# clvrai/mopa-rl

Measured on AMD Instinct MI355X. Metric: valid-state collision checks/sec, higher is better.
Workload: dtype f64; 1 GPU; SawyerPushObstacle-v0 state validity (FK + collision), 4096 envs/GPU x 256 states/env per step, states 50% uniform joint-box samples + 50% near-init N(0,0.3); envs_per_gpu=4096, states_per_env=256, parallelism=env-shard x1

## Files before the change

### mopa_rl_amd/csrc/mopa_hip.hip

```cpp
#include <hip/hip_runtime.h>

#include <algorithm>
#include <cmath>
#include <cstdio>
#include <cstdlib>
#include <cstddef>
#include <cstring>
#include <string>
#include <utility>
#include <vector>

#include <map>
#include <mutex>
#include "../../include/mopa_hip.h"
#include "mopa_device.hpp"
#include "mopa_frames.hpp"
#include "mopa_manifold.hpp"
#include "mopa_sep.hpp"
#include "mopa_fk.hpp"
#include "mopa_host.hpp"
#include "mopa_model_host.hpp"

using namespace mopa;

// ... 154 lines not shown
}
MOPA_D bool wave_any(bool p) { return __ballot(p) != 0ull; }
MOPA_D double wave_min(double v) {
#pragma unroll
    for (int off = 32; off > 0; off >>= 1) {
        double o = __shfl_xor(v, off, 64);
        v = (o < v) ? o : v;
    }
    return v;
}

MOPA_D void tile_ctr_release(unsigned long long *ctr, int lane) {
    if (lane == 0) {
        const unsigned long long done = atomicAdd(ctr + 1, 1ull);
        if (done + 1ull == (unsigned long long)gridDim.x * (blockDim.x >> 6)) {
            atomicExch(ctr, 0ull);
            atomicExch(ctr + 1, 0ull);
        }
    }
}
MOPA_D long long wave_pull64(unsigned long long *ctr, int lane) {
    unsigned long long t = 0ull;
    if (lane == 0) t = atomicAdd(ctr, 1ull);
    const unsigned t_lo = __builtin_amdgcn_readfirstlane((unsigned)t), t_hi = __builtin_amdgcn_readfirstlane((unsigned)(t >> 32));
    return (long long)(((unsigned long long)t_hi << 32) | t_lo);
}
MOPA_D void wave_argmin(double &bd, int &bi) {
#pragma unroll
    for (int off = 32; off > 0; off >>= 1) {
        const double od = __shfl_xor(bd, off, 64);
        const int oi = __shfl_xor(bi, off, 64);
        if (od < bd || (od == bd && oi < bi)) { bd = od; bi = oi; }
    }
}
MOPA_D void row_fill_unused(int32_t *__restrict__ pair, double *__restrict__ dist, long long s, int K, int from, int lane) {
    for (int i = from + lane; i < K; i += 64) {
        pair[s * K + i] = -1;
        dist[s * K + i] = kFar;
    }
}

struct LdsView {
    const double *dbl;
    const int *ints;
    double *grec;
    double *qbuf;
    double *sc;
    unsigned short *wl;
};

MOPA_D void stage_scene(const SceneHdr &h, const double *g_dbl, const int32_t *g_int, double *s_dbl, int *s_int) {
    for (int i = threadIdx.x; i < h.n_dbl; i += blockDim.x) s_dbl[i] = g_dbl[i];
    for (int i = threadIdx.x; i < h.n_int; i += blockDim.x) s_int[i] = g_int[i];
    __syncthreads();
}

MOPA_D LdsView make_view(const SceneHdr &h, unsigned char *smem) {
    LdsView v;
    double *s_dbl = reinterpret_cast<double *>(smem);
    int *s_int = reinterpret_cast<int *>(s_dbl + h.n_dbl);
    int int_pad = (h.n_int + 1) & ~1;
    unsigned char *wave_base = reinterpret_cast<unsigned char *>(s_int + int_pad) + __builtin_amdgcn_readfirstlane((int)(threadIdx.x >> 6)) * h.wave_bytes;
    v.dbl = s_dbl;
    v.ints = s_int;
    v.grec = reinterpret_cast<double *>(wave_base);
    v.qbuf = v.grec + h.nmg * kGeomStride;
    v.sc = v.qbuf + h.na + h.n_pq + h.na;
    v.wl = reinterpret_cast<unsigned short *>(v.sc + 2 * h.nmj);
    return v;
}
MOPA_D LdsView global_view(const double *g_dbl, const int32_t *g_int) {
    LdsView v;
    v.dbl = g_dbl; v.ints = g_int; v.grec = nullptr; v.qbuf = nullptr; v.sc = nullptr; v.wl = nullptr;
    return v;
}

MOPA_D const double *geom_rec(const SceneHdr &h, const LdsView &v, int g) {
    int slot = v.ints[h.o_g_slot + g];
    return (slot >= 0) ? (v.grec + slot * kGeomStride) : (v.dbl + h.o_g_rec + g * kGeomStride);
}

MOPA_D bool pair_culled(const SceneHdr &h, const LdsView &v, int g1, int g2, const double *A, const double *B) {
    const int *I = v.ints;
    const double *D = v.dbl;
    const int t1 = I[h.o_g_type + g1];
    if (bp_cull(A, t1, D[h.o_g_rbound + g1], B, D[h.o_g_rbound + g2])) return true;
    if (t1 == G_PLANE) return false;
    const bool s1 = I[h.o_g_slot + g1] < 0, s2 = I[h.o_g_slot + g2] < 0;
    if (s1 == s2) return false;
    const int gs = s1 ? g1 : g2, gm = s1 ? g2 : g1;
    return aabb_cull(ld3((s1 ? A : B) + GO_POS), D + h.o_g_aabb + 3 * gs, ld3((s1 ? B : A) + GO_POS), D[h.o_g_rbound + gm]);
}
MOPA_D bool pair_culled_band(const SceneHdr &h, const LdsView &v, int g1, int g2, const double *A, const double *B, double band) {
    const int *I = v.ints;
    const double *D = v.dbl;
    const double rba = D[h.o_g_rbound + g1], rbb = D[h.o_g_rbound + g2];
    const V3 diff = sub3(ld3(B + GO_POS), ld3(A + GO_POS));
    if (I[h.o_g_type + g1] == G_PLANE) return dot3(diff, col3(A + GO_MAT, 2)) > rbb + band;
    const double rs = rba + rbb + band;
    if (dot3(diff, diff) > rs * rs) return true;
    const bool s1 = I[h.o_g_slot + g1] < 0, s2 = I[h.o_g_slot + g2] < 0;
    if (s1 == s2) return false;
    return aabb_cull(ld3((s1 ? A : B) + GO_POS), D + h.o_g_aabb + 3 * (s1 ? g1 : g2), ld3((s1 ? B : A) + GO_POS), (s1 ? rbb : rba) + band);
}
struct CullZeroMargin {
    MOPA_D bool operator()(const SceneHdr &h, const LdsView &v, int g1, int g2, const double *A, const double *B) const { return pair_culled(h, v, g1, g2, A, B); }
// ... 660 lines not shown
```

### mopa_rl_amd/csrc/mopa_valid_launch.inc

```

static int64_t k1_lane_min(const MopaScene *S) { return S->k1.v2_forced ? 64 : std::max<int64_t>(64, (int64_t)S->n_cu * 36); }
static int64_t k1_motion_expand_min(const MopaScene *S) { return S->k1.v2_forced ? 64 : std::max<int64_t>(64, (int64_t)S->n_cu * 16); }

using K1FnV1 = decltype(&k_is_valid<false, false>);
using K1FnV2 = decltype(&k_is_valid_v2<false, false>);
using K1FnV5 = decltype(&k_is_valid_v5<false, true, false>);
#define MOPA_K1_COUNT(i_, T_) +1
constexpr int kK1BakedScenes = 0 MOPA_K1_BAKED_SCENES(MOPA_K1_COUNT);
#undef MOPA_K1_COUNT

static K1FnV1 k1_kernel_v1(bool want_md, bool mesh) {
    static const K1FnV1 tab[2][2] = {{k_is_valid<false, false>, k_is_valid<true, false>}, {k_is_valid<false, true>, k_is_valid<true, true>}};
    return tab[mesh][want_md];
}
static K1FnV2 k1_kernel_v2(bool want_md, bool mesh) {
    static const K1FnV2 tab[2][2] = {{k_is_valid_v2<false, false>, k_is_valid_v2<true, false>}, {k_is_valid_v2<false, true>, k_is_valid_v2<true, true>}};
    return tab[mesh][want_md];
}
static K1FnV5 k1_kernel_v5(bool want_md, bool cen_lds, bool gate, int baked) {
    static const K1FnV5 generic[3][2] = {{k_is_valid_v5<false, true, false>, k_is_valid_v5<true, true, false>},
                                         {k_is_valid_v5<false, false, false>, k_is_valid_v5<true, false, false>},
                                         {k_is_valid_v5<false, false, true>, k_is_valid_v5<true, false, true>}};
    if (cen_lds && gate) return nullptr;
    if (!baked) return generic[cen_lds ? 0 : (gate ? 2 : 1)][want_md];
// ... 101 lines not shown
        p.wave = true;
        p.wave_grid = grid_for(S, v2_min);
        p.n_small = v2_min;
    }
    const int64_t tiles = (N + 63) / 64;
    p.blocks = std::min<int64_t>((tiles + kWavesPerBlock - 1) / kWavesPerBlock, (int64_t)S->n_cu * 2);
    p.waves = (size_t)p.blocks * kWavesPerBlock;
    p.v5 = P.use_v5 != 0;
    p.cen_lds = P.v5_cen_lds;
    p.baked = S->k1_baked;
    p.ent_cap = want_md ? P.v5_ent_cap_md : S->hdr.v5_ent_cap;
    if (p.baked) {
        const int ax = k1_baked_axis_words(p.baked) + k1_baked_pair_words(p.baked, want_md);
        if (p.ent_cap - ax >= 256) p.ent_cap -= ax;
        else if (ax > 0) p.baked = 0;
        p.tiles_per_drain = k1_baked_tiles_per_drain(p.baked, want_md);
        if (p.tiles_per_drain > 1) p.pair_tiles = std::max<long long>(0, (long long)tiles - (knobs.pair_tail_set ? std::max<long long>(0, knobs.pair_tail) : (long long)p.waves)) & ~1ll;
    }
    p.lane_lds = !p.v5 ? P.v2_lds_bytes : (want_md ? P.v5_lds_bytes_md : P.v5_lds_bytes);
    p.rows_cap = knobs.rows_cap_set ? knobs.rows_cap : std::min<long long>(std::max<long long>(4096, (long long)N / 2), 1ll << 22);
    p.gate = p.v5 && !p.cen_lds && S->n_mesh_gp > 0;
    p.rows = p.gate && p.rows_cap > 0;
    if (has_n_dev && S->n_mesh_gp > 0 && !p.gate) { p.refusal = "a device-side state count on a scene with mesh pairs needs the gated mesh pass"; return p; }
    p.rows_grid = (unsigned)(knobs.rows_blocks > 0 ? knobs.rows_blocks : 3 * S->n_cu);
    p.rows_lds = (int)((size_t)S->n_mesh_dbl * sizeof(double));
    p.mesh_pass = S->n_mesh_gp > 0;
    p.mesh_lds = P.v2_lds_bytes;
    const unsigned fb = knobs.fb_blocks > 0 ? (unsigned)knobs.fb_blocks : (p.rows ? (unsigned)std::max(1, S->n_cu / 4) : (unsigned)S->n_cu);
    p.mesh_grid = p.gate ? std::min<unsigned>((unsigned)p.blocks, fb) : (unsigned)p.blocks;
    p.debug_mesh = p.gate && knobs.debug_mesh;
    return p;
}

extern "C" int mopa_scene_valid_kernel(const MopaScene *S, int64_t N, char *out, int32_t cap) {
    if (!S || !out || cap < 24) return fail(MOPA_ERR_INVALID_ARG, "null argument / buffer under 24 bytes");
    const K1Plan p = k1_plan(S, N, false, false, false);
    std::snprintf(out, (size_t)cap, "%s", !p.lane ? "k_is_valid" : (p.v5 ? "k_is_valid_v5" : "k_is_valid_v2"));
    return MOPA_OK;
}
extern "C" int mopa_scene_k1_drain_plan(const MopaScene *S, int64_t N, int32_t want_md, int32_t *tiles_per_drain, int32_t *ent_cap) {
    if (!S || !tiles_per_drain || !ent_cap) return fail(MOPA_ERR_INVALID_ARG, "null argument");
    const K1Plan p = k1_plan(S, N, want_md != 0, false, false);
    const bool v5 = p.lane && p.v5;
    *tiles_per_drain = v5 ? p.tiles_per_drain : 0;
    *ent_cap = v5 ? p.ent_cap : 0;
    return MOPA_OK;
}
extern "C" int mopa_scene_motion_kernel(const MopaScene *S, int64_t N, char *out, int32_t cap) {
    if (!S || !out || cap < 24) return fail(MOPA_ERR_INVALID_ARG, "null argument / buffer under 24 bytes");
    std::snprintf(out, (size_t)cap, "%s", S->k1.use_v2 && N >= k1_motion_expand_min(S) ? "k_motion_expand" : "k_check_motion");
    return MOPA_OK;
}

static int launch_is_valid(MopaScene *S, const double *q_active, const double *qpos_env, int64_t N, int64_t samples_per_env,
                           const int *env_idx, uint8_t *valid, double *min_dist, void *stream, const long long *n_dev = nullptr,
                           bool attach = false) {
    if (!S || !valid || (N > 0 && (!q_active || !qpos_env))) return fail(MOPA_ERR_INVALID_ARG, "null argument");
    if (const int rc = state_batch_rule(N, samples_per_env)) return rc;
    if (N == 0) return MOPA_OK;
    ON_DEVICE(S->device);
    hipStream_t st = (hipStream_t)stream;
    if (attach && S->glue_b >= 0) {
        const int rc = glue_attach_scratch(S, qpos_env, (N + samples_per_env - 1) / samples_per_env, st, &qpos_env);
        if (rc) return rc;
    }
    dim3 block(kBlock);
    const K1Plan p = k1_plan(S, N, min_dist != nullptr, env_idx != nullptr, n_dev != nullptr);
    if (p.refusal) return fail(MOPA_ERR_UNSUPPORTED, p.refusal);
    if (p.wave) {
        hipLaunchKernelGGL(k1_kernel_v1(min_dist != nullptr, S->hdr.has_mesh != 0), dim3(p.wave_grid), block, p.wave_lds, st, S->hdr, S->d_dbl, S->d_int, q_active, qpos_env,
                           (long long)N, (long long)samples_per_env, valid, min_dist, env_idx, n_dev, p.lane ? p.n_small : (long long)(1ll << 62));
    }
    if (!p.lane) {
        HIP_TRY(hipGetLastError());
        return MOPA_OK;
    }
    StreamScratch &sc = scratch_for(S, st);
    if (p.waves > sc.slab_waves || (size_t)p.tiles_per_drain > sc.slab_tiles) {
        const size_t want = std::max(std::max(p.waves, sc.slab_waves), (size_t)S->n_cu * 2 * kWavesPerBlock);
        const size_t tiles = std::max((size_t)p.tiles_per_drain, sc.slab_tiles);
        HIP_TRY(grow(S, sc.slab, (want * tiles * (size_t)(S->hdr.nmg + S->hdr.n_save) * kSlabStride + 16) * sizeof(double)));
        HIP_TRY(grow(S, sc.mpr, want * (size_t)kMprCapV5 * kMprRow * sizeof(double)));
        HIP_TRY(grow(S, sc.cen, want * (size_t)S->hdr.nmg * 3 * 64 * sizeof(float)));
        sc.slab_waves = want;
        sc.slab_tiles = tiles;
    }
    if (!sc.k1_ctr.p) {
        HIP_TRY(grow(S, sc.k1_ctr, 64));
        HIP_TRY(hipMemset(sc.k1_ctr.p, 0, 64));
        HIP_TRY(hipStreamSynchronize(nullptr));
    }
    unsigned long long *const d_ctr = sc.k1_ctr.as<unsigned long long>();
    double *const d_slab = sc.slab.as<double>();
    dim3 grid((unsigned)p.blocks);
#ifdef MOPA_V2_PROFILE
    double *d_tail = d_slab + (size_t)p.blocks * kWavesPerBlock * p.tiles_per_drain * (S->hdr.nmg + S->hdr.n_save) * kSlabStride;
    unsigned long long *d_prof = (unsigned long long *)d_tail;
    (void)zero_async(d_prof, 6 * 8, st);
#endif
    long long *mesh_list = nullptr;
    unsigned long long *rows_cnt = nullptr;
    double *mesh_rows = nullptr;
    if (p.gate) {
        HIP_TRY(grow(S, sc.mesh_list, ((size_t)N + 2) * sizeof(long long)));
        rows_cnt = sc.mesh_list.as<unsigned long long>();
        mesh_list = sc.mesh_list.as<long long>() + 1;
        HIP_TRY(zero_async(rows_cnt, 2 * sizeof(long long), st));
        if (p.rows) {
            HIP_TRY(grow(S, sc.mesh_rows, (size_t)p.rows_cap * kMprRow * sizeof(double)));
            mesh_rows = sc.mesh_rows.as<double>();
        }
    }
    if (p.v5) {
        SceneHdr hk = S->hdr;
        hk.v5_ent_cap = p.ent_cap;
        hipLaunchKernelGGL(k1_kernel_v5(min_dist != nullptr, p.cen_lds, p.gate, p.baked), grid, block, p.lane_lds, st, hk, S->d_dbl, S->d_int, S->d_gp_tab, q_active, qpos_env,
                           (long long)N, (long long)samples_per_env, valid, min_dist, d_slab, env_idx, sc.mpr.as<double>(), mesh_list, sc.cen.as<float>(),
                           n_dev, d_ctr, mesh_rows, p.rows_cap, rows_cnt, p.n_small, p.pair_tiles);
        if (p.rows)
            hipLaunchKernelGGL(min_dist ? k_mesh_rows<true> : k_mesh_rows<false>, dim3(p.rows_grid), block, p.rows_lds, st, S->hdr, S->d_dbl, (const double *)mesh_rows,
                               (const unsigned long long *)rows_cnt, p.rows_cap, S->n_mesh_dbl, valid, min_dist);
    } else
        hipLaunchKernelGGL(k1_kernel_v2(min_dist != nullptr, false), grid, block, p.lane_lds, st, S->hdr, S->d_dbl, S->d_int, q_active, qpos_env, (long long)N,
                           (long long)samples_per_env, valid, min_dist, d_slab, 0, env_idx, (const long long *)nullptr, d_ctr);
    if (p.mesh_pass)
        hipLaunchKernelGGL(k1_kernel_v2(min_dist != nullptr, true), dim3(p.mesh_grid), block, p.mesh_lds, st, S->hdr_mesh, S->d_dbl, S->d_int, q_active, qpos_env, (long long)N,
                           (long long)samples_per_env, valid, min_dist, d_slab, 1, env_idx, (const long long *)mesh_list, d_ctr);
    HIP_TRY(hipGetLastError());
    if (p.debug_mesh) {
        long long cnt[2] = {0, 0};
        (void)hipStreamSynchronize(st);
        (void)hipMemcpy(cnt, mesh_list - 1, sizeof(cnt), hipMemcpyDeviceToHost);
        fprintf(stderr, "[mopa] mesh gate: %lld rows handed to k_mesh_rows (cap %lld), %lld of %lld states go to the second pass\n", cnt[0], p.rows_cap, cnt[1], (long long)N);
    }
#ifdef MOPA_V2_PROFILE
    {
        unsigned long long hp[6];
        (void)hipStreamSynchronize(st);
        (void)hipMemcpy(hp, d_prof, 48, hipMemcpyDeviceToHost);
        if (hp[5]) fprintf(stderr, "[v2 profile] per tile cycles: body %.0f geom %.0f cull+push %.0f flush %.0f total %.0f (tiles %llu)\n",
                           (double)hp[0] / hp[5], (double)hp[1] / hp[5], (double)hp[2] / hp[5], (double)hp[3] / hp[5], (double)hp[4] / hp[5], hp[5]);
    }
#endif
    return MOPA_OK;
}

extern "C" int mopa_is_valid_batch(MopaScene *S, const double *q_active, const double *qpos_env, int64_t N,
                                   int64_t samples_per_env, uint8_t *valid, double *min_dist, void *stream) {
    return launch_is_valid(S, q_active, qpos_env, N, samples_per_env, nullptr, valid, min_dist, stream, nullptr, true);
}
extern "C" int mopa_is_valid_batch_counted(MopaScene *S, const double *q_active, const double *qpos_env, int64_t N, int64_t samples_per_env,
// ... 5 lines not shown
```

### mopa_rl_amd/csrc/mopa_valid_v5.inc

```

constexpr int kEntCapV5Max = 1024;
constexpr int kBatCapV5 = 128;
constexpr int kMprCapV5 = 128;
constexpr int kMprRow = 32;
constexpr float kCullEps = 2.0e-5f;

MOPA_D unsigned long long v5_depth_image(double d) { return d != d ? 0x0007ffffffffffffull : f64_sortable(d); }

struct K1Generic {
    static constexpr bool kBaked = false;
    static constexpr int n_ax = 0;
    static constexpr int kTilesPerDrain = 1;
};
#include "mopa_valid_v5_baked.inc"

#ifdef MOPA_V5_TILES_PER_DRAIN
template <class TR, bool WANT_MD> constexpr int k1_tiles_per_drain = TR::kBaked && !WANT_MD ? MOPA_V5_TILES_PER_DRAIN : 1;
#else
template <class TR, bool WANT_MD> constexpr int k1_tiles_per_drain = WANT_MD ? 1 : TR::kTilesPerDrain;
#endif
constexpr unsigned kEntHalfBit = 31;
template <class TR, bool WANT_MD>
constexpr int k1_pair_words_of() {
    constexpr int T = k1_tiles_per_drain<TR, WANT_MD>;
// ... 257 lines not shown
        if constexpr (load == -2) {
            constexpr const unsigned long long *f = TR::fk_sf[sf];
            ppos = V3{k1_bits(f[0]), k1_bits(f[1]), k1_bits(f[2])};
            pquat = Q4{k1_bits(f[3]), k1_bits(f[4]), k1_bits(f[5]), k1_bits(f[6])};
#pragma unroll
            for (int i = 0; i < 9; i++) r.mat[i] = k1_bits(f[7 + i]);
        } else if constexpr (load >= 0) {
            ppos = r.save_pos[load];
            pquat = r.save_quat[load];
            quat2mat(r.mat, pquat);
        } else {
            ppos = r.pos;
            pquat = r.quat;
        }
        const V3 bp{k1_bits(bd[0]), k1_bits(bd[1]), k1_bits(bd[2])};
        const Q4 bq{k1_bits(bd[3]), k1_bits(bd[4]), k1_bits(bd[5]), k1_bits(bd[6])};
        if constexpr (SP) {
            r.pos = k1_offset_s<k1_kind(bd[0]), k1_kind(bd[1]), k1_kind(bd[2])>(ppos, r.mat, bp);
            r.quat = k1_quat_mul_s<k1_kind(bd[3]), k1_kind(bd[4]), k1_kind(bd[5]), k1_kind(bd[6])>(pquat, bq);
        } else {
            r.pos = add3(ppos, mat_vec(r.mat, bp));
            r.quat = quat_mul(pquat, bq);
        }
        if constexpr (jn == 1) {
            const V3 ax{k1_bits(bd[7]), k1_bits(bd[8]), k1_bits(bd[9])}, jp{k1_bits(bd[10]), k1_bits(bd[11]), k1_bits(bd[12])};
            constexpr double ref = k1_bits(bd[13]);
            constexpr int kax = k1_kind(bd[7]), kay = k1_kind(bd[8]), kaz = k1_kind(bd[9]);
            if constexpr (SP && jt == J_HINGE && jp0 && kax == KT_ZERO && kay == KT_ZERO && kaz == KT_ONE) {
                double s1, c1;
                if constexpr (src < TR::na) { s1 = sn[src]; c1 = cs[src]; }
                else mopa_sincos(0.5 * (pv[src - TR::na] - ref), s1, c1);
                r.quat = k1_quat_mul_s<KT_GEN, KT_ZERO, KT_ZERO, KT_GEN>(r.quat, Q4{c1, 0.0, 0.0, s1});
            } else if constexpr (SP && jt == J_SLIDE) {
                double dq;
                if constexpr (src < TR::na) dq = qact[src] - ref;
                else dq = pv[src - TR::na] - ref;
                double jm[9];
                quat2mat(jm, r.quat);
                r.pos = addscl3(r.pos, k1_mat_vec_s<kax, kay, kaz>(jm, ax), dq);
            } else {
                if constexpr (src < TR::na) apply_joint_sc(jt, ax, jp, jp0, qact[src] - ref, sn[src], cs[src], r.pos, r.quat);
                else apply_joint(jt, ax, jp, jp0, pv[src - TR::na] - ref, r.pos, r.quat);
            }
        }
        r.quat = quat_normalize(r.quat);
    }
    quat2mat(r.mat, r.quat);
    if constexpr (save >= 0) {
        r.save_pos[save] = r.pos;
        r.save_quat[save] = r.quat;
    }
    (k1_fk_geom<TR, mgadr + G, SP>(r, sink), ...);
}
template <class TR, bool SPARSE = false, class Sink, int... B>
MOPA_HD bool k1_fk_baked(const double *qa_row, const double *env_row, Sink &sink, std::integer_sequence<int, B...>) {
    static_assert(TR::na <= 8 && TR::n_pq >= 1 && TR::n_save >= 1, "baked walk: at most 8 active values; array sizes padded to 1");
    static_assert(TR::n_res <= kResMax, "baked walk: at most kResMax resident pairs");
    double qact[TR::na], pv[TR::n_pq], sn[TR::na], cs[TR::na];
#pragma unroll
    for (int a = 0; a < TR::na; a++) qact[a] = qa_row[a];
#pragma unroll
    for (int k = 0; k < TR::n_pq; k++) pv[k] = env_row[TR::fk_pq_adr[k]];
#pragma unroll
    for (int a = 0; a < TR::na; a++) mopa_sincos(0.5 * (qact[a] - k1_bits(TR::fk_act_ref[a])), sn[a], cs[a]);
    K1FkRegs<TR> r;
    r.pos = V3{0.0, 0.0, 0.0};
    r.quat = Q4{1.0, 0.0, 0.0, 0.0};
    r.trip = 0u;
    if constexpr (SPARSE) {
#pragma unroll
        for (int a = 0; a < TR::na; a++) r.trip |= !(fabs(qact[a]) <= kSparseInMax) ? 1u : 0u;
#pragma unroll
        for (int k = 0; k < TR::n_pq; k++) r.trip |= !(fabs(pv[k]) <= kSparseInMax) ? 1u : 0u;
        k1_pin(r.trip);
    }
    (k1_fk_body<TR, B, SPARSE>(r, qact, sn, cs, pv, sink, std::make_integer_sequence<int, TR::fk_body[B][4]>{}), ...);
    return r.trip != 0u;
}
template <bool COLD>
struct V5FkSinkT {
    double *slab;
    float *cen;
    MOPA_D void operator()(int m, V3 gp, Q4 gq) {
        double *sp = slab + (size_t)m * kSlabStride;
        if constexpr (COLD) asm volatile("" : "+v"(sp));
        pose7_st<64>(sp, gp, gq);
        float *cp = cen + (size_t)m * 3 * 64;
        cp[0] = (float)gp.x; cp[64] = (float)gp.y; cp[128] = (float)gp.z;
    }
    double res_d[kResMax];
    MOPA_D void resident(int r, double d) { res_d[r] = d; }
    int ax_row;
    MOPA_D void axis(int slot, unsigned word) { reinterpret_cast<unsigned *>(cen)[(ax_row + slot) * 64] = word; }
};
using V5FkSink = V5FkSinkT<false>;

struct V5Lds {
    float *cen;
    unsigned *ent;
    unsigned *bat;
    unsigned *bat2;
    unsigned long long *bad;
    unsigned long long *md;
    bool tp;
};
MOPA_HD int v5_lds_per_wave(int nmg, int ent_cap, bool want_md) { return ((nmg * 3 * 64 * 4) + ent_cap * 4 + 2 * kBatCapV5 * 4 + (want_md ? 64 * 8 : 0) + 8 + 15) & ~15; }

MOPA_D void v5_load_rec2(double (&R1)[15], double (&R2)[15], const SceneHdr &h, const double *D, const double *slab_tile,
                         int gA, int movA, int slotA, int gB, int movB, int slotB, int slA, int slB) {
    const double *sA = D + h.o_g_rec + gA * kGeomStride, *sB = D + h.o_g_rec + gB * kGeomStride;
    double a[7] = {0.0, 0.0, 0.0, 1.0, 0.0, 0.0, 0.0}, b[7] = {0.0, 0.0, 0.0, 1.0, 0.0, 0.0, 0.0};
    if (movA) {
        const double *sp = slab_tile + (size_t)slotA * kSlabStride + slA;
#pragma unroll
        for (int k = 0; k < 7; k++) a[k] = sp[64 * k];
    }
    if (movB) {
        const double *sp = slab_tile + (size_t)slotB * kSlabStride + slB;
#pragma unroll
        for (int k = 0; k < 7; k++) b[k] = sp[64 * k];
    }
#pragma unroll
    for (int i = 0; i < 15; i++) { R1[i] = sA[i]; R2[i] = sB[i]; }
    if (movA) {
        R1[0] = a[0]; R1[1] = a[1]; R1[2] = a[2];
        quat2mat(R1 + GO_MAT, Q4{a[3], a[4], a[5], a[6]});
    }
    if (movB) {
        R2[0] = b[0]; R2[1] = b[1]; R2[2] = b[2];
        quat2mat(R2 + GO_MAT, Q4{b[3], b[4], b[5], b[6]});
    }
}

template <bool WANT_MD, int T = 1>
MOPA_D int v5_flush(const SceneHdr &h, const LdsView &v, const V5Lds &q, const int *s_tab, const double *slab_tile, int lane,
                    int head, int n, int code, int stage = 0, int head2 = 0, int count2 = 0, double *mpr_ring = nullptr,
                    int mpr_head = 0, int *mpr_count = nullptr, long long tile_base = 0) {
    bool to_mpr = false;
    unsigned e = 0;
// ... 72 lines not shown

template <bool WANT_MD, int T = 1>
MOPA_D void v5_drain(const SceneHdr &h, const LdsView &v, const V5Lds &q, const int *s_tab, const double *slab_tile, int lane,
                     int n_ent, unsigned present, double *mpr_ring, int mpr_head, int *mpr_count, long long tile_base) {
    wave_sync();
    for (int code = 0; code < PC_COUNT; code++) {
        if (!((present >> code) & 1u)) continue;
        int head = 0, count = 0, head2 = 0, count2 = 0;
        for (int base = 0; base < n_ent; base += 64) {
            const int i = base + lane;
            bool take = false;
            unsigned e = 0;
            if (i < n_ent) {
                e = q.ent[i];
                take = (int)((e >> 12) & 0xf) == code;
                if (!WANT_MD) take = take && !((q.bad[T > 1 ? e >> kEntHalfBit : 0u] >> (e & 63)) & 1ull);
            }
            const unsigned long long mask = __ballot(take);
            if (!mask) continue;
            if (take) q.bat[(head + count + __popcll(mask & ((1ull << lane) - 1ull))) & (kBatCapV5 - 1)] = e;
            count += __popcll(mask);
            if (count >= 64) {
                wave_sync();
                if (code == PC_CONVEX) {
                    count2 += v5_flush<WANT_MD, T>(h, v, q, s_tab, slab_tile, lane, head, 64, code, 1, head2, count2, mpr_ring, mpr_head, mpr_count, tile_base);
                    if (count2 >= 64) {
                        v5_flush<WANT_MD, T>(h, v, q, s_tab, slab_tile, lane, head2, 64, code, 2);
                        head2 = (head2 + 64) & (kBatCapV5 - 1);
                        count2 -= 64;
                    }
                } else {
                    v5_flush<WANT_MD, T>(h, v, q, s_tab, slab_tile, lane, head, 64, code);
                }
                head = (head + 64) & (kBatCapV5 - 1);
                count -= 64;
            }
        }
        if (count > 0) {
            wave_sync();
            if (code == PC_CONVEX) count2 += v5_flush<WANT_MD, T>(h, v, q, s_tab, slab_tile, lane, head, count, code, 1, head2, count2, mpr_ring, mpr_head, mpr_count, tile_base);
            else v5_flush<WANT_MD, T>(h, v, q, s_tab, slab_tile, lane, head, count, code);
        }
        if (code == PC_CONVEX) {
            while (count2 > 0) {
                const int nb = count2 < 64 ? count2 : 64;
                v5_flush<WANT_MD, T>(h, v, q, s_tab, slab_tile, lane, head2, nb, code, 2);
                head2 = (head2 + nb) & (kBatCapV5 - 1);
                count2 -= nb;
            }
        }
    }
}

template <bool WANT_MD, bool CEN_LDS, bool GATE, class TR = K1Generic>
__global__ __launch_bounds__(kBlock, TR::kBaked ? 2 : 1) void k_is_valid_v5(SceneHdr h, const double *__restrict__ g_dbl, const int32_t *__restrict__ g_int,
                                                         const int32_t *__restrict__ g_tab, const double *__restrict__ q_active,
                                                         const double *__restrict__ qpos_env, long long N, long long samples_per_env,
                                                         unsigned char *__restrict__ valid, double *__restrict__ min_dist,
                                                         double *__restrict__ slab_all, const int *__restrict__ env_idx , double *__restrict__ mpr_all,
                                                         long long *__restrict__ mesh_list ,
                                                         float *__restrict__ cen_all ,
                                                         const long long *__restrict__ n_dev , unsigned long long *__restrict__ tile_ctr,
                                                         double *__restrict__ mesh_rows ,
                                                         long long mesh_rows_cap, unsigned long long *__restrict__ mesh_rows_cnt,
                                                         long long n_small ,
                                                         long long pair_tiles ) {
    constexpr int T = k1_tiles_per_drain<TR, WANT_MD>;
    static_assert(T == 1 || (T == 2 && TR::kBaked), "pair drain: two tiles, baked scenes only (the generic phase 0 borrows the entry buffer)");
    if constexpr (T > 1) static_assert(TR::padr[TR::nmg - 1] + TR::pnum[TR::nmg - 1] < (1 << 15), "pair drain: the entry's table index leaves bit 31 to the half");
    if (n_dev) {
        const long long nd = *n_dev;
        if (nd < N) N = nd;
        if (nd < n_small) N = 0;
    }
    extern __shared__ __attribute__((aligned(16))) unsigned char smem[];
    double *s_dbl = reinterpret_cast<double *>(smem);
    int *s_int = reinterpret_cast<int *>(s_dbl + h.n_dbl);
    int *s_tab = s_int + ((h.n_int + 3) & ~3);
    constexpr int kTail = GATE ? 3 : 1;
    for (int i = threadIdx.x; i < 8 * h.n_gp + kTail * h.nmg; i += blockDim.x) s_tab[i] = g_tab[i];
    stage_scene(h, g_dbl, g_int, s_dbl, s_int);
    LdsView v;
    v.dbl = s_dbl; v.ints = s_int; v.grec = nullptr; v.qbuf = nullptr; v.sc = nullptr; v.wl = nullptr;
    const int lane = threadIdx.x & 63, wave = threadIdx.x >> 6;
    V5Lds q;
    {
        const int n_cen = CEN_LDS ? h.nmg : 0;
        int ent_words = h.v5_ent_cap;
        if constexpr (k1_axis_words<TR> > 0) ent_words += k1_axis_words<TR>;
        if constexpr (T > 1) ent_words += k1_pair_words<TR, WANT_MD>;
        unsigned char *base = reinterpret_cast<unsigned char *>(s_tab + ((8 * h.n_gp + kTail * h.nmg + 3) & ~3)) + wave * v5_lds_per_wave(n_cen, ent_words, WANT_MD);
        q.cen = reinterpret_cast<float *>(base);
        q.ent = reinterpret_cast<unsigned *>(q.cen + n_cen * 3 * 64);
        if constexpr (k1_axis_words<TR> > 0) q.ent += k1_axis_words<TR>;
        q.bat = q.ent + h.v5_ent_cap;
        q.bat2 = q.bat + kBatCapV5;
        q.md = reinterpret_cast<unsigned long long *>(q.bat2 + kBatCapV5);
        q.bad = WANT_MD ? q.md + 64 * T : q.md;
        q.tp = false;
    }
    const double *__restrict__ GD = g_dbl;
    const int32_t *__restrict__ GI = g_int;
    const int nslab = h.nmg + h.n_save;
    double *slab = slab_all + ((size_t)blockIdx.x * kWavesPerBlock + wave) * (size_t)(T * nslab) * kSlabStride + lane;
    const double *slab_tile = slab - lane;
    double *mpr_ring = mpr_all + ((size_t)blockIdx.x * kWavesPerBlock + wave) * (size_t)kMprCapV5 * kMprRow;
    float *gcen = CEN_LDS ? nullptr : cen_all + ((size_t)blockIdx.x * kWavesPerBlock + wave) * (size_t)h.nmg * 3 * 64 + lane;
    int mpr_head = 0, mpr_count = 0;
    const long long n_tiles = (N + 63) >> 6;
    for (;;) {
        long long tile = 0;
        if (lane == 0) tile = (long long)atomicAdd(tile_ctr, (unsigned long long)T);
        tile = __shfl(tile, 0, 64);
        bool single = false;
        if constexpr (T > 1) {
            if (tile >= pair_tiles) {
                tile = pair_tiles + ((tile - pair_tiles) >> 1);
                single = true;
            }
        }
        const bool fin = tile >= n_tiles;
        if (!fin) {
        int n_ent;
        unsigned present;
        long long s;
        bool act, need_mesh;
        int hf = 0;
#pragma unroll 1
        do {
        if (T > 1 && hf > 0 && (single || tile + hf >= n_tiles)) break;
        s = (tile + hf) * 64 + lane;
        act = s < N;
        if (!act) s = N - 1;
        const double *qa_row = q_active + s * h.na;
        const double *env_row = qpos_env + (env_idx ? (long long)env_idx[s] : s / samples_per_env) * h.nq;
        if (lane == 0) q.bad[hf] = 0ull;
        if (WANT_MD) q.md[64 * hf + lane] = f64_sortable(0.0);

        double res_d[kResMax] = {};
#ifdef MOPA_V5_FK_REPS
        for (int fk_rep = 0; fk_rep < MOPA_V5_FK_REPS; fk_rep++)
#endif
        if constexpr (TR::kBaked) {
            double *fk_slab = T > 1 ? slab + (size_t)hf * (size_t)nslab * kSlabStride : slab;
            asm volatile("" : "+v"(fk_slab));
            V5FkSink sink{fk_slab, q.cen + lane, {}, 3 * TR::nmg};
            if constexpr (k1_sparse_on<TR>) {
                const bool fk_trip = k1_fk_baked<TR, true>(qa_row, env_row, sink, std::make_integer_sequence<int, TR::nmb>{});
                if (__builtin_expect(__ballot(fk_trip) != 0ull, 0)) {
                    const double *qa_cold = qa_row, *env_cold = env_row;
                    asm volatile("" : "+v"(qa_cold), "+v"(env_cold) : : "memory");
                    V5FkSinkT<true> cold{fk_slab, q.cen + lane, {}, 3 * TR::nmg};
                    k1_fk_baked<TR>(qa_cold, env_cold, cold, std::make_integer_sequence<int, TR::nmb>{});
#pragma unroll
                    for (int r = 0; r < kResMax; r++) sink.res_d[r] = cold.res_d[r];
                }
            } else {
                k1_fk_baked<TR>(qa_row, env_row, sink, std::make_integer_sequence<int, TR::nmb>{});
            }
#pragma unroll
            for (int r = 0; r < kResMax; r++) res_d[r] = sink.res_d[r];
#ifdef MOPA_V5_FK_REPS
            asm volatile("" ::: "memory");
#endif
        } else {
            double *ps = reinterpret_cast<double *>(q.ent);
            bool tile_poses = false;
            if (!GATE && h.n_pas_b > 0) {
                const unsigned long long er = (unsigned long long)env_row;
                const unsigned long long e0 = ((unsigned long long)(unsigned)__builtin_amdgcn_readfirstlane((int)(er >> 32)) << 32) | (unsigned)__builtin_amdgcn_readfirstlane((int)(unsigned)er);
                tile_poses = __all(er == e0);
            }
            q.tp = !GATE && tile_poses;
            if (!GATE && tile_poses) {
                for (int lv = 0; lv < h.n_pas_lv; lv++) {
                    const int i = s_int[h.o_pas_lv + lv] + lane;
                    if (i < s_int[h.o_pas_lv + lv + 1]) {
                        const int b = s_int[h.o_pas_b + i];
                        const int *ri = s_int + h.o_mbr + 8 * b;
                        V2BodyI bi;
                        bi.jn = ri[0]; bi.jntadr = ri[1]; bi.load = ri[2]; bi.sf = ri[3]; bi.save = ri[4]; bi.mgadr = ri[5]; bi.mgnum = ri[6]; bi.jt_qsrc = ri[7];
                        const double *bd = s_dbl + h.o_mbd + 16 * b;
                        const int jt0 = bi.jt_qsrc & 0x7f, qsrc0 = bi.jt_qsrc >> 8;
                        V3 pos;
                        Q4 quat;
                        if (bi.jn == 1 && jt0 == J_FREE) {
                            const double *qp = env_row + s_int[h.o_pq_adr + (qsrc0 - h.na)];
                            fk_free_step(qp, pos, quat);
                        } else {
                            V3 ppos;
                            Q4 pquat;
                            double mat[9];
                            const int par = s_int[h.o_mb_parent + b];
                            if (par < 0) {
                                sf_frame_ld(h, s_dbl, bi.sf, ppos, pquat, mat);
                            } else {
                                const double *pp = ps + 7 * (s_int[h.o_mb_pas + par] & 0xffff);
                                pose7_ld<1>(pp, ppos, pquat);
                                quat2mat(mat, pquat);
                            }
                            pos = add3(ppos, mat_vec(mat, ld3(bd)));
                            quat = quat_mul(pquat, Q4{bd[3], bd[4], bd[5], bd[6]});
                            for (int jj = 0; jj < bi.jn; jj++) {
                                V3 ax, jp;
                                double ref;
                                int jt, src;
// ... 301 lines not shown
                }
                if (sv) q.ent[n_ent + __builtin_amdgcn_mbcnt_hi((unsigned)(mask >> 32), __builtin_amdgcn_mbcnt_lo((unsigned)mask, 0u))] =
                            (unsigned)lane | ((unsigned)m << 6) | (pcode << 12) | ((unsigned)(p0 + k) << 16) | (T > 1 ? (unsigned)hf << kEntHalfBit : 0u);
                n_ent += __popcll(mask);
                present |= 1u << pcode;
#ifdef MOPA_V5_KO_DRAIN
                if (n_ent > h.v5_ent_cap - 64) n_ent = 0;
#endif
                if (n_ent > h.v5_ent_cap - 64) {
                    v5_drain<WANT_MD, T>(h, v, q, s_tab, slab_tile, lane, n_ent, present, mpr_ring, mpr_head, &mpr_count, tile * 64);
                    n_ent = 0;
                    present = 0u;
                }
            };
            if constexpr (TR::kBaked) {
                for (unsigned long long bits = any_kept; bits; bits &= bits - 1ull) pass_b_pair((int)__builtin_ctzll(bits));
            } else {
                for (int k = 0; k < pn; k++) pass_b_pair(k);
            }
        }
        } while (T > 1 && ++hf < T);
#ifndef MOPA_V5_KO_DRAIN
        if (n_ent > 0) v5_drain<WANT_MD, T>(h, v, q, s_tab, slab_tile, lane, n_ent, present, mpr_ring, mpr_head, &mpr_count, tile * 64);
#endif
        wave_sync();
        if constexpr (T == 1) {
            if (act) {
                valid[s] = ((*q.bad >> lane) & 1ull) ? 0 : 1;
                if (WANT_MD) min_dist[s] = f64_unsortable(q.md[lane]);
            }
        } else {
#pragma unroll
            for (int ho = 0; ho < T; ho++) {
                const long long so = (tile + ho) * 64 + lane;
                if (so < N && !(ho > 0 && single)) {
                    const int hf = ho;
                    valid[so] = ((q.bad[hf] >> lane) & 1ull) ? 0 : 1;
                    if (WANT_MD) min_dist[so] = f64_unsortable(q.md[64 * hf + lane]);
                }
            }
        }
        if (GATE && mesh_list) {
            const bool f = act && need_mesh;
            const unsigned long long fm = __ballot(f);
            if (fm) {
                unsigned long long at = 0;
                if (lane == 0) at = atomicAdd(reinterpret_cast<unsigned long long *>(mesh_list), (unsigned long long)__popcll(fm));
                at = __shfl(at, 0, 64);
                if (f) mesh_list[1 + at + __popcll(fm & ((1ull << lane) - 1ull))] = s;
            }
        }
        wave_sync();
        }
        while (mpr_count >= 64 || (fin && mpr_count > 0)) {
            const int nb = mpr_count < 64 ? mpr_count : 64;
            __threadfence_block();
            v5_mpr_rows<WANT_MD>(h, mpr_ring, mpr_head, nb, lane, valid, min_dist);
            mpr_head = (mpr_head + nb) & (kMprCapV5 - 1);
            mpr_count -= nb;
        }
        if (fin) break;
    }
    tile_ctr_release(tile_ctr, lane);
}

#ifndef MOPA_MESH_ROWS_G
#define MOPA_MESH_ROWS_G 8
#endif
template <bool WANT_MD, int G = MOPA_MESH_ROWS_G>
__global__ __launch_bounds__(kBlock) void k_mesh_rows(SceneHdr h, const double *__restrict__ g_dbl, const double *__restrict__ rows,
                                                       const unsigned long long *__restrict__ cnt, long long cap, int n_mesh_dbl,
                                                       unsigned char *__restrict__ valid, double *__restrict__ min_dist) {
    extern __shared__ __attribute__((aligned(16))) unsigned char smem[];
    double *s_mesh = reinterpret_cast<double *>(smem);
    long long n = (long long)*cnt;
    if (n > cap) n = cap;
    if (n == 0) return;
    for (int i = threadIdx.x; i < n_mesh_dbl; i += blockDim.x) s_mesh[i] = g_dbl[h.o_mesh + i];
    __syncthreads();
    const double *aux = s_mesh - h.o_mesh;
    const int lane = threadIdx.x & 63;
    const long long gw = (long long)blockIdx.x * kWavesPerBlock + (threadIdx.x >> 6), nw = (long long)gridDim.x * kWavesPerBlock;
    constexpr int kPer = 64 / G;
    for (long long base = gw * kPer; base < n; base += nw * kPer) {
        const long long i = base + lane / G;
        if (i < n) {
            const double *row = rows + (size_t)i * kMprRow;
            double R1[15], R2[15];
#pragma unroll
            for (int k = 0; k < 15; k++) { R1[k] = row[k]; R2[k] = row[15 + k]; }
            const long long s = __double_as_longlong(row[30]);
            const int tt = (int)__double_as_longlong(row[31]);
            const double d = geom_dist<true, G>((tt >> 16) & 0xf, R1, tt & 0xff, R2, (tt >> 8) & 0xff, aux);
            if ((lane & (G - 1)) == 0) {
                if (d <= h.thr) valid[s] = 0;
                if (WANT_MD && d < 0.0) atomicMax(reinterpret_cast<unsigned long long *>(min_dist + s), (unsigned long long)__double_as_longlong(d));
            }
        }
    }
}
```

Baseline: 2.591 billion checks/s.

## Stage only needed scene data in baked K1 kernel and use global address space for slab

For baked scenes, the v5 validity kernel now stages into LDS only the geometry records, geom types, moving-geom indices and one table column, not the whole scene and table. This cuts per-block prologue work. The FK slab stores and the cold-path input pointers are also marked as global address space so the compiler can emit global rather than flat memory instructions, and pose stores are written out explicitly. An optional timeline instrumentation path is added behind a compile flag. Skipping staging risks missing data if any baked code path reads other LDS fields.

```diff
diff --git a/mopa_rl_amd/csrc/mopa_hip.hip b/mopa_rl_amd/csrc/mopa_hip.hip
--- a/mopa_rl_amd/csrc/mopa_hip.hip
+++ b/mopa_rl_amd/csrc/mopa_hip.hip
@@ -230,6 +230,14 @@
 MOPA_D void stage_scene(const SceneHdr &h, const double *g_dbl, const int32_t *g_int, double *s_dbl, int *s_int) {
     for (int i = threadIdx.x; i < h.n_dbl; i += blockDim.x) s_dbl[i] = g_dbl[i];
     for (int i = threadIdx.x; i < h.n_int; i += blockDim.x) s_int[i] = g_int[i];
+    __syncthreads();
+}
+
+MOPA_D void stage_scene_k1_baked(const SceneHdr &h, const double *g_dbl, const int32_t *g_int, const int32_t *g_tab, double *s_dbl, int *s_int, int *s_tab) {
+    for (int i = threadIdx.x; i < h.ng * kGeomStride; i += blockDim.x) s_dbl[h.o_g_rec + i] = g_dbl[h.o_g_rec + i];
+    for (int i = threadIdx.x; i < h.ng; i += blockDim.x) s_int[h.o_g_type + i] = g_int[h.o_g_type + i];
+    for (int i = threadIdx.x; i < h.nmg; i += blockDim.x) s_int[h.o_mg_geom + i] = g_int[h.o_mg_geom + i];
+    for (int i = threadIdx.x; i < h.n_gp; i += blockDim.x) s_tab[8 * i + 7] = g_tab[8 * i + 7];
     __syncthreads();
 }
 
diff --git a/mopa_rl_amd/csrc/mopa_valid_launch.inc b/mopa_rl_amd/csrc/mopa_valid_launch.inc
--- a/mopa_rl_amd/csrc/mopa_valid_launch.inc
+++ b/mopa_rl_amd/csrc/mopa_valid_launch.inc
@@ -177,6 +177,20 @@
     return MOPA_OK;
 }
 
+#ifdef MOPA_V5_TIMELINE
+constexpr size_t kK1TimelineWords = kTlRow;
+static unsigned long long *g_k1_timeline = nullptr;
+static long long g_k1_timeline_rows = 0;
+extern "C" long long mopa_k1_timeline_read(unsigned long long *out, long long cap_rows) {
+    if (!out || !g_k1_timeline || hipDeviceSynchronize() != hipSuccess) return -1;
+    const long long n = std::min(cap_rows, g_k1_timeline_rows);
+    if (n > 0 && hipMemcpy(out, g_k1_timeline, (size_t)n * kTlRow * 8, hipMemcpyDeviceToHost) != hipSuccess) return -1;
+    return n;
+}
+#else
+constexpr size_t kK1TimelineWords = 0;
+#endif
+
 static int launch_is_valid(MopaScene *S, const double *q_active, const double *qpos_env, int64_t N, int64_t samples_per_env,
                            const int *env_idx, uint8_t *valid, double *min_dist, void *stream, const long long *n_dev = nullptr,
                            bool attach = false) {
@@ -204,7 +218,7 @@
     if (p.waves > sc.slab_waves || (size_t)p.tiles_per_drain > sc.slab_tiles) {
         const size_t want = std::max(std::max(p.waves, sc.slab_waves), (size_t)S->n_cu * 2 * kWavesPerBlock);
         const size_t tiles = std::max((size_t)p.tiles_per_drain, sc.slab_tiles);
-        HIP_TRY(grow(S, sc.slab, (want * tiles * (size_t)(S->hdr.nmg + S->hdr.n_save) * kSlabStride + 16) * sizeof(double)));
+        HIP_TRY(grow(S, sc.slab, (want * tiles * (size_t)(S->hdr.nmg + S->hdr.n_save) * kSlabStride + 16 + want * kK1TimelineWords) * sizeof(double)));
         HIP_TRY(grow(S, sc.mpr, want * (size_t)kMprCapV5 * kMprRow * sizeof(double)));
         HIP_TRY(grow(S, sc.cen, want * (size_t)S->hdr.nmg * 3 * 64 * sizeof(float)));
         sc.slab_waves = want;
@@ -222,6 +236,11 @@
     double *d_tail = d_slab + (size_t)p.blocks * kWavesPerBlock * p.tiles_per_drain * (S->hdr.nmg + S->hdr.n_save) * kSlabStride;
     unsigned long long *d_prof = (unsigned long long *)d_tail;
     (void)zero_async(d_prof, 6 * 8, st);
+#endif
+#ifdef MOPA_V5_TIMELINE
+    g_k1_timeline = reinterpret_cast<unsigned long long *>(d_slab + (size_t)p.blocks * kWavesPerBlock * p.tiles_per_drain * (S->hdr.nmg + S->hdr.n_save) * kSlabStride);
+    g_k1_timeline_rows = p.v5 ? (long long)p.waves : 0;
+    HIP_TRY(zero_async(g_k1_timeline, p.waves * (size_t)kTlRow * 8, st));
 #endif
     long long *mesh_list = nullptr;
     unsigned long long *rows_cnt = nullptr;
diff --git a/mopa_rl_amd/csrc/mopa_valid_v5.inc b/mopa_rl_amd/csrc/mopa_valid_v5.inc
--- a/mopa_rl_amd/csrc/mopa_valid_v5.inc
+++ b/mopa_rl_amd/csrc/mopa_valid_v5.inc
@@ -333,8 +333,8 @@
     }
     (k1_fk_geom<TR, mgadr + G, SP>(r, sink), ...);
 }
-template <class TR, bool SPARSE = false, class Sink, int... B>
-MOPA_HD bool k1_fk_baked(const double *qa_row, const double *env_row, Sink &sink, std::integer_sequence<int, B...>) {
+template <class TR, bool SPARSE = false, class QP, class Sink, int... B>
+MOPA_HD bool k1_fk_baked(QP qa_row, QP env_row, Sink &sink, std::integer_sequence<int, B...>) {
     static_assert(TR::na <= 8 && TR::n_pq >= 1 && TR::n_save >= 1, "baked walk: at most 8 active values; array sizes padded to 1");
     static_assert(TR::n_res <= kResMax, "baked walk: at most kResMax resident pairs");
     double qact[TR::na], pv[TR::n_pq], sn[TR::na], cs[TR::na];
@@ -358,14 +358,22 @@
     (k1_fk_body<TR, B, SPARSE>(r, qact, sn, cs, pv, sink, std::make_integer_sequence<int, TR::fk_body[B][4]>{}), ...);
     return r.trip != 0u;
 }
+#ifdef MOPA_V5_FLAT_SLAB
+typedef double k1_gdouble;
+typedef const double k1_gcdouble;
+#else
+typedef __attribute__((address_space(1))) double k1_gdouble;
+typedef const __attribute__((address_space(1))) double k1_gcdouble;
+#endif
 template <bool COLD>
 struct V5FkSinkT {
-    double *slab;
+    k1_gdouble *slab;
     float *cen;
     MOPA_D void operator()(int m, V3 gp, Q4 gq) {
-        double *sp = slab + (size_t)m * kSlabStride;
+        k1_gdouble *sp = slab + (size_t)m * kSlabStride;
         if constexpr (COLD) asm volatile("" : "+v"(sp));
-        pose7_st<64>(sp, gp, gq);
+        sp[0] = gp.x; sp[64] = gp.y; sp[2 * 64] = gp.z;
+        sp[3 * 64] = gq.w; sp[4 * 64] = gq.x; sp[5 * 64] = gq.y; sp[6 * 64] = gq.z;
         float *cp = cen + (size_t)m * 3 * 64;
         cp[0] = (float)gp.x; cp[64] = (float)gp.y; cp[128] = (float)gp.z;
     }
@@ -544,6 +552,38 @@
     }
 }
 
+constexpr int kTlRow = 64, kTlPulls = kTlRow - 10;
+#ifdef MOPA_V5_TIMELINE
+#define V5_TL_DECL const unsigned long long tl_t0 = __builtin_amdgcn_s_memrealtime();
+#define V5_TL_STAGED const unsigned long long tl_t1 = __builtin_amdgcn_s_memrealtime();
+#define V5_TL_ROW(tail_, w_)                                                                                  \
+    unsigned long long *const tl_row = reinterpret_cast<unsigned long long *>(tail_) + (w_) * (size_t)kTlRow; \
+    unsigned tl_pulls = 0u, tl_tiles = 0u;                                                                    \
+    if (lane == 0) { tl_row[0] = tl_t0; tl_row[1] = tl_t1; tl_row[9] = (unsigned long long)__builtin_amdgcn_s_getreg(4 | (31 << 11)) | ((unsigned long long)__builtin_amdgcn_s_getreg(20 | (3 << 11)) << 32); }
+#define V5_TL_PULL(fin_)                                                                  \
+    {                                                                                     \
+        const unsigned long long tl_t = __builtin_amdgcn_s_memrealtime();                 \
+        if (lane == 0) {                                                                  \
+            if (tl_pulls < (unsigned)kTlPulls) tl_row[10 + tl_pulls] = tl_t;              \
+            tl_row[(fin_) ? 4 : 3] = tl_t;                                                \
+        }                                                                                 \
+        tl_pulls++;                                                                       \
+    }
+#define V5_TL_TILE tl_tiles++;
+#define V5_TL_MPR0(fin_, n_) if ((fin_) && lane == 0) tl_row[7] = (unsigned long long)(n_);
+#define V5_TL_MPR1(fin_) if ((fin_) && lane == 0) tl_row[5] = __builtin_amdgcn_s_memrealtime();
+#define V5_TL_EXIT if (lane == 0) { tl_row[2] = tl_pulls; tl_row[8] = tl_tiles; tl_row[6] = __builtin_amdgcn_s_memrealtime(); }
+#else
+#define V5_TL_DECL
+#define V5_TL_STAGED
+#define V5_TL_ROW(tail_, w_)
+#define V5_TL_PULL(fin_)
+#define V5_TL_TILE
+#define V5_TL_MPR0(fin_, n_)
+#define V5_TL_MPR1(fin_)
+#define V5_TL_EXIT
+#endif
+
 template <bool WANT_MD, bool CEN_LDS, bool GATE, class TR = K1Generic>
 __global__ __launch_bounds__(kBlock, TR::kBaked ? 2 : 1) void k_is_valid_v5(SceneHdr h, const double *__restrict__ g_dbl, const int32_t *__restrict__ g_int,
                                                          const int32_t *__restrict__ g_tab, const double *__restrict__ q_active,
@@ -565,13 +605,22 @@
         if (nd < N) N = nd;
         if (nd < n_small) N = 0;
     }
+    V5_TL_DECL
     extern __shared__ __attribute__((aligned(16))) unsigned char smem[];
     double *s_dbl = reinterpret_cast<double *>(smem);
     int *s_int = reinterpret_cast<int *>(s_dbl + h.n_dbl);
     int *s_tab = s_int + ((h.n_int + 3) & ~3);
     constexpr int kTail = GATE ? 3 : 1;
-    for (int i = threadIdx.x; i < 8 * h.n_gp + kTail * h.nmg; i += blockDim.x) s_tab[i] = g_tab[i];
-    stage_scene(h, g_dbl, g_int, s_dbl, s_int);
+#ifndef MOPA_V5_FULL_STAGING
+    if constexpr (TR::kBaked) {
+        stage_scene_k1_baked(h, g_dbl, g_int, g_tab, s_dbl, s_int, s_tab);
+    } else
+#endif
+    {
+        for (int i = threadIdx.x; i < 8 * h.n_gp + kTail * h.nmg; i += blockDim.x) s_tab[i] = g_tab[i];
+        stage_scene(h, g_dbl, g_int, s_dbl, s_int);
+    }
+    V5_TL_STAGED
     LdsView v;
     v.dbl = s_dbl; v.ints = s_int; v.grec = nullptr; v.qbuf = nullptr; v.sc = nullptr; v.wl = nullptr;
     const int lane = threadIdx.x & 63, wave = threadIdx.x >> 6;
@@ -600,6 +649,7 @@
     float *gcen = CEN_LDS ? nullptr : cen_all + ((size_t)blockIdx.x * kWavesPerBlock + wave) * (size_t)h.nmg * 3 * 64 + lane;
     int mpr_head = 0, mpr_count = 0;
     const long long n_tiles = (N + 63) >> 6;
+    V5_TL_ROW(slab_all + (size_t)gridDim.x * kWavesPerBlock * (size_t)(T * nslab) * kSlabStride, (size_t)blockIdx.x * kWavesPerBlock + wave)
     for (;;) {
         long long tile = 0;
         if (lane == 0) tile = (long long)atomicAdd(tile_ctr, (unsigned long long)T);
@@ -612,6 +662,7 @@
             }
         }
         const bool fin = tile >= n_tiles;
+        V5_TL_PULL(fin)
         if (!fin) {
         int n_ent;
         unsigned present;
@@ -621,6 +672,7 @@
 #pragma unroll 1
         do {
         if (T > 1 && hf > 0 && (single || tile + hf >= n_tiles)) break;
+        V5_TL_TILE
         s = (tile + hf) * 64 + lane;
         act = s < N;
         if (!act) s = N - 1;
@@ -636,14 +688,15 @@
         if constexpr (TR::kBaked) {
             double *fk_slab = T > 1 ? slab + (size_t)hf * (size_t)nslab * kSlabStride : slab;
             asm volatile("" : "+v"(fk_slab));
-            V5FkSink sink{fk_slab, q.cen + lane, {}, 3 * TR::nmg};
+            k1_gdouble *const fk_slab_g = (k1_gdouble *)fk_slab;
+            V5FkSink sink{fk_slab_g, q.cen + lane, {}, 3 * TR::nmg};
             if constexpr (k1_sparse_on<TR>) {
                 const bool fk_trip = k1_fk_baked<TR, true>(qa_row, env_row, sink, std::make_integer_sequence<int, TR::nmb>{});
                 if (__builtin_expect(__ballot(fk_trip) != 0ull, 0)) {
                     const double *qa_cold = qa_row, *env_cold = env_row;
                     asm volatile("" : "+v"(qa_cold), "+v"(env_cold) : : "memory");
-                    V5FkSinkT<true> cold{fk_slab, q.cen + lane, {}, 3 * TR::nmg};
-                    k1_fk_baked<TR>(qa_cold, env_cold, cold, std::make_integer_sequence<int, TR::nmb>{});
+                    V5FkSinkT<true> cold{fk_slab_g, q.cen + lane, {}, 3 * TR::nmg};
+                    k1_fk_baked<TR>((k1_gcdouble *)qa_cold, (k1_gcdouble *)env_cold, cold, std::make_integer_sequence<int, TR::nmb>{});
 #pragma unroll
                     for (int r = 0; r < kResMax; r++) sink.res_d[r] = cold.res_d[r];
                 }
@@ -1051,6 +1104,7 @@
         }
         wave_sync();
         }
+        V5_TL_MPR0(fin, mpr_count)
         while (mpr_count >= 64 || (fin && mpr_count > 0)) {
             const int nb = mpr_count < 64 ? mpr_count : 64;
             __threadfence_block();
@@ -1058,9 +1112,11 @@
             mpr_head = (mpr_head + nb) & (kMprCapV5 - 1);
             mpr_count -= nb;
         }
+        V5_TL_MPR1(fin)
         if (fin) break;
     }
     tile_ctr_release(tile_ctr, lane);
+    V5_TL_EXIT
 }
 
 #ifndef MOPA_MESH_ROWS_G
```

After: 2.633 billion checks/s, median of 6. +1.6%, better.
